# pinellolab/GRAFIMO

Measured on AMD Instinct MI355X. Metric: scored haplotype k-mers/sec, higher is better.
Workload: dtype int32

## Files before the change

### grafimo_amd/csrc/gfm_graph_fused.hpp

```cpp

constexpr int kMaxMM = 3;
struct GraphHit { int tile, score; long long q2k; };
constexpr int kHitWinShift = 56;
constexpr long long kHitWalkMask = (1ll << kHitWinShift) - 1;
struct Tile {
    long long p0, limit;
    int n_win, region;
    int i_lo, i_hi;
    int w_base, i_far;
};
constexpr int kTilePure = 1 << 8;
struct DelWin { int tile_k, i0; };
constexpr int kDelTileBits = 25;
__device__ __forceinline__ int del_tile(const DelWin &d) { return d.tile_k & ((1 << kDelTileBits) - 1); }
__device__ __forceinline__ int del_k(const DelWin &d) { return (int)((unsigned)d.tile_k >> kDelTileBits); }
struct HeavyWin {
    int tile_k, i0;
    int ns;
    unsigned item_base, n_chunks, rounds_per_chunk;
    long long walks;
    long long q_base;
    int jx, del_len;
};
constexpr long long kHeavyWalks = 64;
// ... 181 lines not shown

struct WinInfo {
    int i0, ns;
    long long walks;
    bool listed, simple;
    long long walks_b;
    int ns_b, jx, del_len;
};
template <class S>
__device__ __forceinline__ WinInfo classify_window(const GraphDev &g, const S &sites, long long p, int W, long long limit,
                                                   int i_lo, int i_hi)
{
    int lo = i_lo, hi = i_hi;
    while (lo < hi) {
        const int mid = (lo + hi) >> 1;
        if (sites.at(mid).pos < p) lo = mid + 1; else hi = mid;
    }
    WinInfo w{lo, 0, 1, false, false, 0, 0, 0, 0};
    bool over = false;
    const bool covered = g.n_dels > 0 && sites.covered(p, lo);
    w.listed = covered;
    int n_indel = 0, first_indel = -1;
    for (int i = lo;; ++i, ++w.ns) {
        const SiteRec r = sites.at(i);
        if (r.pos >= p + W) break;
        if (r.del_len || r.ins_len) {
            w.listed = true;
            if (n_indel++ == 0) first_indel = i;
        } else if (!over) {
            w.walks *= 1 + (r.n_alts & 3);
            over = w.walks > kFusedMaxWalks;
        }
    }
    bool ins_before = false;
    if (g.n_ins > 0) {
        for (int k = lo - 1; k >= i_lo; --k) {
            const SiteRec r = sites.at(k);
            if (r.pos != p - 1) break;
            if (r.ins_len > 0) { w.listed = true; ins_before = true; }
        }
        if (!w.listed && p + W > limit) { w.walks = 0; over = false; }
    }
    if (p + W > g.ref_len && !w.listed) w.walks = 0;
    if (w.listed && !covered && !ins_before && n_indel == 1 && !over) {
        const SiteRec d = sites.at(first_indel);
        if (d.del_len > 0) {
            const long long x = d.pos, len = d.del_len;
            bool ok = true, over_b = false;
            long long wb = 1;
            int nsb = 0;
            for (int i = lo;; ++i, ++nsb) {
                const SiteRec r = sites.at(i);
                if (r.pos >= p + W + len) break;
                if (r.del_len || r.ins_len) { if (i != first_indel) { ok = false; break; } continue; }
                if (r.pos > x && r.pos <= x + len) continue;
                if (!over_b) { wb *= 1 + (r.n_alts & 3); over_b = wb > kFusedMaxWalks; }
            }
            if (ok && !over_b) {
                w.simple = true;
                w.ns_b = nsb;
                w.jx = (int)(x - p);
                w.del_len = (int)len;
                const bool a_lives = p + W <= limit && p + W <= g.ref_len;
                const bool b_lives = a_lives && w.jx < W - 1 && p + W + len <= limit && p + W + len <= g.ref_len;
                if (!a_lives) w.walks = 0;
                w.walks_b = b_lives ? wb : 0;
                return w;
            }
        }
    }
    if (w.listed) w.walks = 0;
    else if (over) w.walks = -1;
    return w;
}

constexpr int kWaveQueue = 96;
constexpr int kOwnerSlots = 256;
template <int MM, bool LISTING, bool GENERAL> struct WaveLdsT {
    SiteRec rec[kWaveSites];
    uint2 winfo[kTileWin];
    unsigned wsc[MM][kTileWin];
    unsigned short incl[kTileWin];
    unsigned char owner[kOwnerSlots];
    unsigned char ref[kWaveRefBytes];
    int reach[GENERAL ? kWaveSites : 1];
    unsigned score_b[MM][GENERAL ? kTileWin : 1];
    unsigned sinfo[GENERAL ? kTileWin : 1];
    DelWin queue[(LISTING && GENERAL) ? kWaveQueue : 1];
};
__host__ __device__ constexpr int fused_tab_dwords(int MM, int W) { return (MM * W * 8 + 3) & ~3; }

#ifndef GFM_GRAPH_SCORE_MIN_WAVES
#define GFM_GRAPH_SCORE_MIN_WAVES 6
#endif
template <int MM, bool LISTING, bool GENERAL>
__global__ void __launch_bounds__(kFusedMaxWaves * 64, LISTING ? 1 : GFM_GRAPH_SCORE_MIN_WAVES)
graph_score_kernel(GraphDev g, FusedArgs a, const Tile *__restrict__ tiles, int tile_begin, int n_tiles,
                   DelWin *__restrict__ del_wins, int *__restrict__ del_count, int *__restrict__ overflow,
                   HeavyWin *__restrict__ heavy_wins, unsigned long long *__restrict__ heavy_ctl, int *__restrict__ plan_overflow_w)
{
    using WL = WaveLdsT<MM, LISTING, GENERAL>;
    extern __shared__ __attribute__((aligned(16))) unsigned char fused_lds[];
    const int W = a.W, W8 = W * 8;
    const int nw = (int)(blockDim.x >> 6), n_thr = (int)blockDim.x;
    unsigned *tab = reinterpret_cast<unsigned *>(fused_lds);
    WL *wl0 = reinterpret_cast<WL *>(tab + fused_tab_dwords(MM, W));
    WL *wl = wl0 + (threadIdx.x >> 6);
    unsigned long long *blk_rows = reinterpret_cast<unsigned long long *>(wl0 + nw);
    int *blk_q = reinterpret_cast<int *>(blk_rows + nw);
    unsigned *h = reinterpret_cast<unsigned *>(blk_q + nw + 4);
    const int tid = threadIdx.x, lane = tid & 63, wave = __builtin_amdgcn_readfirstlane(tid >> 6);
    int *next_tile = blk_q + nw + 1;
    unsigned long long rows_done = 0;
    int q_n = 0;
    unsigned long long acc_t[6] = {0, 0, 0, 0, 0, 0}, acc_n = 0;
#ifdef GFM_LAB
    unsigned ph_t[5] = {0, 0, 0, 0, 0};
#endif
    auto lap = [&](int slot, unsigned long long &t0) {
#ifdef GFM_LAB
        if (a.tile_log) {
            const unsigned long long t1 = wall_clock64();
            if (slot < 5) ph_t[slot] = (unsigned)(t1 - t0);
            t0 = t1;
            return;
        }
#endif
        if (!GFM_DBG(a)) return;
        const unsigned long long t1 = wall_clock64();
        acc_t[slot] += t1 - t0;
        t0 = t1;
    };
    static_assert(kWaveSites <= 64, "one staged record per lane");
    struct TilePf { SiteRec r0; int reach0; unsigned long long refw; };
    auto issue = [&](const Tile &t) {
        TilePf f{};
        const int staged = min(t.i_far - t.i_lo + 1, kWaveSites);
        if (lane < staged) {
            f.r0 = packed_site(g, t.i_lo + lane);
            if constexpr (GENERAL) {
                if (g.n_dels > 0 && !(t.n_win & kTilePure)) {
                    const int i = t.i_lo + lane;
                    const long long r = (i <= g.n_sites ? g.max_reach[i] : -1ll) - t.p0;
                    f.reach0 = (int)max(-1ll, min(r, 0x7fffffffll));
                }
            }
        }
        if (lane < kWaveRefBytes / 8) {
            const long long at = t.p0 + 8 * lane;
            unsigned long long v = 0x4e4e4e4e4e4e4e4eull;
            if (at + 8 <= g.ref_len + (long long)kReadPad) v = load_u64(g.ref + at);
            if (at + 8 > g.ref_len)
                for (int b = 0; b < 8; ++b)
                    if (at + b >= g.ref_len) v = (v & ~(0xffull << (8 * b))) | (0x4eull << (8 * b));
            f.refw = v;
        }
        return f;
    };
    auto commit = [&](const Tile &t, const TilePf &f) {
        const int staged = min(t.i_far - t.i_lo + 1, kWaveSites);
        if (lane < staged) {
            wl->rec[lane] = f.r0;
            if constexpr (GENERAL) wl->reach[lane] = f.reach0;
        }
        if (lane < kWaveRefBytes / 8) *reinterpret_cast<unsigned long long *>(wl->ref + 8 * lane) = f.refw;
    };
    auto tile_at = [&](int j) -> int {
        const long long at = (long long)tile_begin + (long long)blockIdx.x + (long long)j * (long long)gridDim.x;
        return at < (long long)n_tiles ? (int)at : n_tiles;
    };
    auto claim = [&]() -> int {
        int j = 0;
        if (lane == 0) j = atomicAdd(next_tile, 1);
        return tile_at(__builtin_amdgcn_readfirstlane(j));
    };
    static_assert(sizeof(Tile) == 40, "ten dwords");
    auto tile_ask = [&](int idx) -> unsigned {
        return lane < 10 ? reinterpret_cast<const unsigned *>(tiles + idx)[lane] : 0u;
    };
    auto tile_take = [&](unsigned dw) -> Tile {
        unsigned v[10];
#pragma unroll
        for (int k = 0; k < 10; ++k) v[k] = (unsigned)__builtin_amdgcn_readlane((int)dw, k);
        Tile t;
        t.p0 = (long long)(((unsigned long long)v[1] << 32) | v[0]);
        t.limit = (long long)(((unsigned long long)v[3] << 32) | v[2]);
        t.n_win = (int)v[4]; t.region = (int)v[5]; t.i_lo = (int)v[6]; t.i_hi = (int)v[7]; t.w_base = (int)v[8]; t.i_far = (int)v[9];
        return t;
    };
    Tile t_cur{}, t_nxt{};
    TilePf pf{};
    int ti = tile_at(wave), ti1 = n_tiles, ti2 = n_tiles;
    unsigned nxt_dw = ti < n_tiles ? tile_ask(ti) : 0u;
#pragma unroll
    for (int m = 0; m < MM; ++m)
        for (int i = tid; i < W8; i += n_thr) tab[m * W8 + i] = a.tab[m][i];
    for (int i = tid; i < a.slab_stride; i += n_thr) h[i] = 0u;
    if (tid == 0) { *next_tile = nw; next_tile[1] = 0; }
    if (ti < n_tiles) {
        t_cur = tile_take(nxt_dw);
        pf = issue(t_cur);
    }
    __syncthreads();
#ifndef GFM_GRAPH_HOLD1
    if (ti < n_tiles) {
        ti1 = claim();
        if (ti1 < n_tiles) nxt_dw = tile_ask(ti1);
    }
#endif
#ifdef GFM_LAB
    const unsigned long long dbg_t0 = a.tile_log ? wall_clock64() : 0ull;
#endif
    for (; ti < n_tiles; ti = ti1, ti1 = ti2) {
#ifdef GFM_LAB
        const unsigned long long tl_begin = a.tile_log ? wall_clock64() : 0ull;
#endif
#ifdef GFM_LAB
        unsigned long long tk0 = (GFM_DBG(a) || a.tile_log) ? wall_clock64() : 0ull, tk_tile = tk0;
#else
        unsigned long long tk0 = 0ull, tk_tile = 0ull;
#endif
        const Tile t = t_cur;
        commit(t, pf);
        const int my_pos = pf.r0.pos, my_alts = pf.r0.n_alts;
        __builtin_amdgcn_wave_barrier();
        ti2 = n_tiles;
#ifndef GFM_GRAPH_HOLD1
        if (ti1 < n_tiles) {
            t_nxt = tile_take(nxt_dw);
            pf = issue(t_nxt);
            t_cur = t_nxt;
            ti2 = claim();
            if (ti2 < n_tiles) nxt_dw = tile_ask(ti2);
        }
#else
        ti1 = claim();
        if (ti1 < n_tiles) nxt_dw = tile_ask(ti1);
#endif
        const int staged = min(t.i_far - t.i_lo + 1, kWaveSites);
        const int n_win = t.n_win & 0xff;
        lap(0, tk0);
        auto work = [&](const auto &sites, auto pure_tag) {
        constexpr bool PURE = decltype(pure_tag)::value;
        auto ref_at = [&](long long x) -> unsigned {
            const long long d = x - t.p0;
            if ((unsigned long long)d < (unsigned long long)kWaveRefBytes) return (unsigned)wl->ref[d];
            ColdArgs ka = cold_args();
            return x < ka->g.ref_len ? (unsigned)ka->g.ref[x] : (unsigned)'N';
        };
        const long long p = t.p0 + lane;
        bool listed = false;
        int i0 = t.i_lo, ns = 0, ns_b = 0, jx = 0, dlen = 0;
        int walks_a = 0, walks_b = 0;
        auto to_heavy = [&](long long n_walks, long long q_base, int ns_, int jx_, int del_len_) {
            if (!a.listing) return;
            const long long rounds = (n_walks + 63) >> 6;
            const unsigned n_chunks = (unsigned)min((long long)kHeavyMaxChunks, (rounds + kHeavyItemRounds - 1) / kHeavyItemRounds);
            ColdArgs ka = cold_args();
            const unsigned long long got = atomicAdd(ka->heavy_ctl, (1ull << 32) | (unsigned long long)n_chunks);
            const unsigned slot = (unsigned)(got >> 32), base = (unsigned)(got & 0xffffffffull);
            if (slot < (unsigned)kHeavyCap && (unsigned long long)base + n_chunks < 0xffffffffull) {
                ka->heavy_wins[slot] = HeavyWin{ti | (lane << kDelTileBits), i0, ns_, base, n_chunks,
                                            (unsigned)((rounds + n_chunks - 1) / n_chunks), n_walks, q_base, jx_, del_len_};
            } else {
                atomicMax(ka->overflow, 1);
                atomicMax(ka->plan_overflow_w, 1);
            }
        };
        if constexpr (PURE) {
            const int pi = (int)p, n_t = t.i_hi - t.i_lo;
            int before = 0, inside = 0;
            unsigned long long prod = 1;
            for (int s = 0; s < n_t; ++s) {
                const int spos = __builtin_amdgcn_readlane(my_pos, s);
                const int na = __builtin_amdgcn_readlane(my_alts, s) & 3;
                const bool bef = spos < pi, in = !bef && spos < pi + W;
                before += bef ? 1 : 0;
                inside += in ? 1 : 0;
                if (in && prod <= (unsigned long long)kFusedMaxWalks) prod *= (unsigned long long)(1 + na);
            }
            if (lane < n_win && !GFM_LAB_BIT(a, 4)) {
                i0 = t.i_lo + before;
                ns = inside;
                long long wlk = (p + W <= t.limit && p + W <= g.ref_len) ? (long long)prod : 0ll;
                if (wlk > kFusedMaxWalks) { atomicMax(cold_args()->overflow, 1); wlk = 0; }
                else if (wlk > kHeavyWalks) { to_heavy(wlk, 0, ns, 0, 0); wlk = 0; }
                walks_a = (int)wlk;
            }
        } else if (lane < n_win && !GFM_LAB_BIT(a, 4)) {
            WinInfo wi = classify_window(g, sites, p, W, t.limit, t.i_lo, t.i_hi);
            if (wi.walks < 0) { atomicMax(cold_args()->overflow, 1); wi.walks = 0; }
            i0 = wi.i0;
            if (wi.simple && (wi.ns_b > 255 || wi.del_len > 0xffff)) {
                wi.simple = false;
                wi.walks = 0;
                wi.walks_b = 0;
            }
            if (wi.i0 - t.i_lo > 0xffff) { atomicMax(cold_args()->overflow, 1); wi.walks = 0; wi.walks_b = 0; wi.listed = wi.simple = false; }
            const bool many = wi.walks + wi.walks_b > kHeavyWalks;
            if (wi.simple && many) {
                if (wi.ns <= 64 && wi.ns_b <= 64) {
                    if (wi.walks > 0) to_heavy(wi.walks, 0, wi.ns, 0, 0);
                    if (wi.walks_b > 0) to_heavy(wi.walks_b, wi.walks, wi.ns_b, wi.jx, wi.del_len);
                    wi.listed = false;
                } else {
                    wi.simple = false;
                }
                wi.walks = 0;
                wi.walks_b = 0;
            }
            listed = wi.listed && !wi.simple;
            if (!wi.listed && !wi.simple && many && wi.ns <= 64) {
                to_heavy(wi.walks, 0, wi.ns, 0, 0);
                wi.walks = 0;
            }
            ns = wi.ns; ns_b = wi.ns_b; jx = wi.jx; dlen = wi.del_len;
            walks_a = (int)wi.walks;
            walks_b = (int)wi.walks_b;
        }
        if (GFM_LAB_BIT(a, 4) && lane < n_win) walks_a = 1;
        lap(1, tk0);
        unsigned sc_a[MM];
#pragma unroll
        for (int m = 0; m < MM; ++m) sc_a[m] = 0u;
        int bad_a = 0;
        if (lane < n_win) {
            if (walks_a > 0 && !GFM_LAB_BIT(a, 2)) {
                int bad = 0;
                int j = 0;
                for (; j + 4 <= W; j += 4) {
                    unsigned c[4];
#pragma unroll
                    for (int u = 0; u < 4; ++u) c[u] = base_code(wl->ref[lane + j + u]);
#pragma unroll
                    for (int m = 0; m < MM; ++m) {
                        unsigned v[4];
#pragma unroll
                        for (int u = 0; u < 4; ++u) v[u] = tab[m * W8 + (j + u) * 8 + c[u]];
                        sc_a[m] += (v[0] + v[1]) + (v[2] + v[3]);
                    }
                    bad += (int)((c[0] >> 2) + (c[1] >> 2) + (c[2] >> 2) + (c[3] >> 2));
                }
                for (; j < W; ++j) {
                    const unsigned c = base_code(wl->ref[lane + j]);
#pragma unroll
                    for (int m = 0; m < MM; ++m) sc_a[m] += tab[m * W8 + j * 8 + c];
                    bad += (int)(c >> 2);
                }
                bad_a = bad;
            }
            if constexpr (!PURE) if (walks_b > 0) {
                unsigned sum[MM];
#pragma unroll
                for (int m = 0; m < MM; ++m) sum[m] = 0u;
                int bad = 0;
                if (lane + W + dlen <= kWaveRefBytes) {
                    const unsigned char *rb = wl->ref + lane;
                    int j = 0;
                    for (; j + 4 <= W; j += 4) {
                        unsigned c[4];
#pragma unroll
                        for (int u = 0; u < 4; ++u) c[u] = base_code(rb[j + u + (j + u > jx ? dlen : 0)]);
#pragma unroll
                        for (int m = 0; m < MM; ++m) {
                            unsigned v[4];
#pragma unroll
                            for (int u = 0; u < 4; ++u) v[u] = tab[m * W8 + (j + u) * 8 + c[u]];
                            sum[m] += (v[0] + v[1]) + (v[2] + v[3]);
                        }
                        bad += (int)((c[0] >> 2) + (c[1] >> 2) + (c[2] >> 2) + (c[3] >> 2));
                    }
                    for (; j < W; ++j) {
                        const unsigned c = base_code(rb[j + (j > jx ? dlen : 0)]);
#pragma unroll
                        for (int m = 0; m < MM; ++m) sum[m] += tab[m * W8 + j * 8 + c];
                        bad += (int)(c >> 2);
                    }
                } else {
                    for (int j = 0; j < W; ++j) {
                        const unsigned c = base_code(ref_at(p + j + (j > jx ? dlen : 0)));
#pragma unroll
                        for (int m = 0; m < MM; ++m) sum[m] += tab[m * W8 + j * 8 + c];
                        bad += (int)(c >> 2);
                    }
                }
#pragma unroll
                for (int m = 0; m < MM; ++m) wl->score_b[m][lane] = sum[m];
                wl->sinfo[lane] = (unsigned)bad | ((unsigned)jx << 8) | ((unsigned)dlen << 16);
            }
        }
        lap(2, tk0);
        {
            const bool has_ref = walks_a > 0;
            if (!GFM_LAB_BIT(a, 8)) {
#pragma unroll
                for (int m = 0; m < MM; ++m) {
                    const int s_f = bad_a ? a.min_val[m] : (int)(sc_a[m] & 0xffffu);
                    const int s_r = bad_a ? a.min_val[m] : (int)(sc_a[m] >> 16);
                    if (a.hnb[m] > 0) {
                        book_score_cold(a, m, h, has_ref, s_f);
                        if (!a.forward_only) book_score_cold(a, m, h, has_ref, s_r);
                    }
                    push_hits_cold(m, has_ref && s_f >= a.cutoff[m], ti, lane, 0, s_f);
                    if (!a.forward_only) push_hits_cold(m, has_ref && s_r >= a.cutoff[m], ti, lane, 1, s_r);
                }
            }
            rows_done += (unsigned long long)__popcll(__builtin_amdgcn_ballot_w64(has_ref)) * (a.forward_only ? 1ull : 2ull);
        }
        if constexpr (LISTING && !PURE) {
            const unsigned long long lm = __builtin_amdgcn_ballot_w64(listed);
            if (lm) {
                if (listed) wl->queue[q_n + __popcll(lm & ((1ull << lane) - 1ull))] = DelWin{ti | (lane << kDelTileBits), i0};
                q_n += __popcll(lm);
                if (q_n >= kWaveQueue - kTileWin) {
                    int base = 0;
                    if (lane == 0) base = atomicAdd(cold_args()->del_count, q_n);
                    base = __builtin_amdgcn_readfirstlane(base);
                    __builtin_amdgcn_wave_barrier();
                    { DelWin *dw = cold_args()->del_wins; for (int i = lane; i < q_n; i += 64) dw[base + i] = wl->queue[i]; }
                    q_n = 0;
                }
            }
        }
        const int nA = walks_a > 0 ? walks_a - 1 : 0;
        const int v_w = nA + walks_b;
        const int incl = wave_prefix_sum(v_w);
        int total = __builtin_amdgcn_readlane(incl, 63);
        if (GFM_LAB_BIT(a, 1)) total = 0;
        const bool owners = total < kOwnerSlots;
        if (total > 0) {
            wl->incl[lane] = (unsigned short)incl;
            if (owners)
                for (int x = incl - v_w; x < incl; ++x) wl->owner[x] = (unsigned char)lane;
            wl->winfo[lane] = uint2{(unsigned)(i0 - t.i_lo) | ((unsigned)ns << 16) | ((unsigned)ns_b << 24),
                                    (unsigned)bad_a | ((unsigned)walks_a << 7) | ((unsigned)(incl - v_w) << 14)};
#pragma unroll
            for (int m = 0; m < MM; ++m) wl->wsc[m][lane] = sc_a[m];
        }
        __builtin_amdgcn_wave_barrier();
        lap(3, tk0);
#ifdef GFM_GRAPH_HOLD1
        if (ti1 < n_tiles) {
            t_nxt = tile_take(nxt_dw);
            pf = issue(t_nxt);
            t_cur = t_nxt;
        }
#endif
        for (int base = 0; base < total; base += 64) {
            const int wt = base + lane;
            const bool live = wt < total;
            int k = 0;
            long long q = 0;
            unsigned sum[MM];
#pragma unroll
            for (int m = 0; m < MM; ++m) sum[m] = 0u;
            int bad = 0;
            if (live) {
                if (owners) {
                    k = wl->owner[wt];
                } else {
                    int lo = 0, hi = kTileWin - 1;
                    while (lo < hi) {
                        const int mid = (lo + hi) >> 1;
                        if ((int)wl->incl[mid] > wt) hi = mid; else lo = mid + 1;
                    }
                    k = lo;
                }
                const uint2 pw = wl->winfo[k];
                const int qq = wt - (int)(pw.y >> 14);
                const int wa = (int)((pw.y >> 7) & 0x7fu);
                const int nA_k = wa > 0 ? wa - 1 : 0;
                const bool jump = qq >= nA_k;
                const int i0k = t.i_lo + (int)(pw.x & 0xffffu);
                if (!jump) {
                    q = qq + 1;
#pragma unroll
                    for (int m = 0; m < MM; ++m) sum[m] = wl->wsc[m][k];
                    bad = (int)(pw.y & 0x7fu);
                    unsigned rest = (unsigned)q;
                    const int pk = (int)(t.p0 + k);
                    for (int s = (int)((pw.x >> 16) & 0xffu) - 1; s >= 0 && rest; --s) {
                        const SiteRec r = sites.at(i0k + s);
                        const int nall = (r.del_len | r.ins_len) ? 1 : 1 + (r.n_alts & 3);
                        const int al = take_digit32(rest, nall);
                        if (al) {
                            const int j = r.pos - pk;
                            const unsigned cr = base_code(wl->ref[k + j]), ca = base_code((unsigned)r.n_alts >> (8 * al));
#pragma unroll
                            for (int m = 0; m < MM; ++m) sum[m] += tab[m * W8 + j * 8 + ca] - tab[m * W8 + j * 8 + cr];
                            bad += (int)(ca >> 2) - (int)(cr >> 2);
                        }
                    }
                } else if constexpr (!PURE) {
                    q = (long long)wa + (qq - nA_k);
#pragma unroll
                    for (int m = 0; m < MM; ++m) sum[m] = wl->score_b[m][k];
                    const unsigned si = wl->sinfo[k];
                    bad = (int)(si & 0xffu);
                    unsigned rest = (unsigned)(qq - nA_k);
                    const long long pk = t.p0 + k;
                    const long long x = pk + (long long)((si >> 8) & 0xffu), len = (long long)(si >> 16);
                    for (int s = (int)(pw.x >> 24) - 1; s >= 0 && rest; --s) {
                        const SiteRec r = sites.at(i0k + s);
                        if (r.del_len | r.ins_len) continue;
                        if (r.pos > x && r.pos <= x + len) continue;
                        const int nall = 1 + (r.n_alts & 3);
                        const int al = take_digit32(rest, nall);
                        if (al) {
                            const int j = (int)(r.pos - pk) - (r.pos > x ? (int)len : 0);
                            const unsigned cr = base_code(ref_at(r.pos)), ca = base_code((unsigned)r.n_alts >> (8 * al));
#pragma unroll
                            for (int m = 0; m < MM; ++m) sum[m] += tab[m * W8 + j * 8 + ca] - tab[m * W8 + j * 8 + cr];
                            bad += (int)(ca >> 2) - (int)(cr >> 2);
                        }
                    }
                }
            }
            if (GFM_LAB_BIT(a, 8)) continue;
#pragma unroll
            for (int m = 0; m < MM; ++m) {
                const int s_f = bad ? a.min_val[m] : (int)(sum[m] & 0xffffu);
                const int s_r = bad ? a.min_val[m] : (int)(sum[m] >> 16);
                if (a.hnb[m] > 0) {
                    book_score_cold(a, m, h, live, s_f);
                    if (!a.forward_only) book_score_cold(a, m, h, live, s_r);
                }
                push_hits_cold(m, live && s_f >= a.cutoff[m], ti, k, 2 * q, s_f);
                if (!a.forward_only) push_hits_cold(m, live && s_r >= a.cutoff[m], ti, k, 2 * q + 1, s_r);
            }
        }
        rows_done += (unsigned long long)total * (a.forward_only ? 1ull : 2ull);
        };
        if constexpr (!GENERAL) {
            work(LdsTileSites{wl->rec, nullptr, t.p0, t.i_lo}, std::true_type{});
        } else {
            if (t.n_win & kTilePure) work(LdsTileSites{wl->rec, wl->reach, t.p0, t.i_lo}, std::true_type{});
            else if (t.i_far - t.i_lo + 1 <= kWaveSites) work(LdsTileSites{wl->rec, wl->reach, t.p0, t.i_lo}, std::false_type{});
            else {
                const GraphDev g_far = ((const ScoreKernArgs *)cold_args())->g;
                work(TileSites{g_far, wl->rec, wl->reach, t.p0, t.i_lo, staged}, std::false_type{});
            }
        }
        __builtin_amdgcn_wave_barrier();
        lap(4, tk0);
        lap(5, tk_tile);
#ifdef GFM_LAB
        if (a.tile_log && lane == 0 && !a.listing) {
            a.tile_log[ti] = (((wall_clock64() - tl_begin) & 0xffffffull) << 40) | (((tl_begin - dbg_t0) & 0xffffffull) << 16) | (blockIdx.x & 0xffffu);
            unsigned long long w = 0;
            for (int k = 0; k < 5; ++k) w |= (unsigned long long)min(ph_t[k], 4095u) << (12 * k);
            a.tile_log[n_tiles + ti] = w;
        }
#endif
        ++acc_n;
    }
    if (const int lw_items = cold_args()->a.lw_items; lw_items > 0) {
        ColdArgs ka = cold_args();
        const int n16 = ka->a.lw_pitch >> 4;
        for (;;) {
            int j = 0;
            if (lane == 0) j = atomicAdd(next_tile + 1, 1);
            const long long it = (long long)blockIdx.x + (long long)__builtin_amdgcn_readfirstlane(j) * (long long)gridDim.x;
            if (it >= (long long)lw_items) break;
            const size_t row = (size_t)it * 64 + (size_t)lane;
            const LwMeta me = ka->a.lw_meta[row];
            const bool live = me.tile_k >= 0;
            uint4 v[4];
#pragma unroll
            for (int c = 0; c < 4; ++c) v[c] = (c < n16 && live) ? ka->a.lw_kmers[row * (size_t)n16 + c] : uint4{0x41414141u, 0x41414141u, 0x41414141u, 0x41414141u};
            unsigned sum[MM];
#pragma unroll
            for (int m = 0; m < MM; ++m) sum[m] = 0u;
            int bad = 0;
#pragma unroll
            for (int c = 0; c < 4; ++c) {
                if (16 * c >= W) break;
                const unsigned dw[4] = {v[c].x, v[c].y, v[c].z, v[c].w};
#pragma unroll
                for (int u = 0; u < 16; ++u) {
                    const int jj = 16 * c + u;
                    if (jj < W) {
                        const unsigned cd = base_code((dw[u >> 2] >> (8 * (u & 3))) & 0xffu);
#pragma unroll
                        for (int m = 0; m < MM; ++m) sum[m] += tab[m * W8 + jj * 8 + cd];
                        bad += (int)(cd >> 2);
                    }
                }
            }
            const int w_tile = me.tile_k & ((1 << kDelTileBits) - 1), w_k = (int)((unsigned)me.tile_k >> kDelTileBits);
#pragma unroll
            for (int m = 0; m < MM; ++m) {
                const int s_f = bad ? a.min_val[m] : (int)(sum[m] & 0xffffu);
                const int s_r = bad ? a.min_val[m] : (int)(sum[m] >> 16);
                if (a.hnb[m] > 0) {
                    book_score_cold(a, m, h, live, s_f);
                    if (!a.forward_only) book_score_cold(a, m, h, live, s_r);
                }
                push_hits_cold(m, live && s_f >= a.cutoff[m], w_tile, w_k, 2 * me.q0, s_f);
                if (!a.forward_only) push_hits_cold(m, live && s_r >= a.cutoff[m], w_tile, w_k, 2 * me.q0 + 1, s_r);
            }
            rows_done += (unsigned long long)__popcll(__builtin_amdgcn_ballot_w64(live)) * (a.forward_only ? 1ull : 2ull);
        }
    }
    if (unsigned long long *dbg = GFM_DBG(a); dbg && lane == 0 && acc_n)
        for (int k = 0; k < 6; ++k) {
            atomicAdd(&dbg[8 + k], acc_t[k]);
            atomicMax(&dbg[24 + k], acc_t[k]);
            atomicAdd(&dbg[40 + k], acc_n);
        }
    if (lane == 0) { blk_rows[wave] = rows_done; blk_q[wave] = q_n; }
    __syncthreads();
    if (tid == 0) {
        if (!a.listing && blockIdx.x == 0 && *cold_args()->a.plan_overflow) atomicMax(cold_args()->overflow, 1);
        unsigned long long rows = 0;
        int left = 0;
        for (int k = 0; k < nw; ++k) { rows += blk_rows[k]; left += blk_q[k]; }
        if (rows) atomicAdd(cold_args()->a.n_rows, rows);
        blk_q[nw] = left ? atomicAdd(cold_args()->del_count, left) : 0;
    }
    __syncthreads();
    if constexpr (LISTING && GENERAL) {
        int at = blk_q[nw];
        for (int k = 0; k < wave; ++k) at += blk_q[k];
        { DelWin *dw = cold_args()->del_wins; for (int i = lane; i < q_n; i += 64) dw[at + i] = wl->queue[i]; }
    }
    { unsigned *slabs = cold_args()->a.slabs; for (int i = tid; i < a.slab_stride; i += n_thr) slabs[(size_t)blockIdx.x * a.slab_stride + i] = h[i]; }
}

struct ScoreEmit {
    const uint8_t *alt_bases, *ins_bases;
    const int *ins_off;
    uint8_t *fwd;
    int *src;
    static constexpr bool kWantsBases = true;
    __device__ void base(int j, long long x, int snp, int a, int)
    {
        src[j] = (int)x;
        if (snp >= 0 && a) { fwd[j] = alt_bases[(size_t)snp * kMaxAlts + (a - 1)]; src[j] = -1; }
    }
    __device__ void ins_base(int j, int site, int t) { fwd[j] = ins_bases[ins_off[site] + t]; src[j] = -1; }
    __device__ void took(int) {}
    __device__ void passed(int) {}
};


struct DelBatchRec {
    long long incl;
    int n_lay, pad;
    LayoutRec lay[kFusedLayouts];
};
struct DelItem { int batch, chunk, n_chunks, pad; };
constexpr int kDelItemRounds = 1, kDelMaxItems = 64;
constexpr int kDelExtraItems = 1 << 20, kDelMaxChunks = 1 << 18;

__global__ void __launch_bounds__(kFusedDelThreads)
graph_del_count_kernel(GraphDev g, int W, const Tile *__restrict__ tiles, const DelWin *__restrict__ del_wins,
                       const int *__restrict__ del_count, int *__restrict__ overflow, int *__restrict__ plan_overflow,
                       DelBatchRec *__restrict__ recs, DelItem *__restrict__ items, int *__restrict__ item_count,
                       int *__restrict__ extra_used, int *__restrict__ long_items)
{
    extern __shared__ __attribute__((aligned(16))) unsigned char fused_lds[];
    constexpr int T = kFusedDelThreads;
    SiteRec *cache = reinterpret_cast<SiteRec *>(fused_lds);
    const int lane = threadIdx.x;
    const int n_listed = *del_count;
    for (int batch = blockIdx.x; (long long)batch * T < n_listed; batch += gridDim.x) {
        __syncthreads();
        const int m = batch * T + lane;
        long long walks = 0;
        DelBatchRec rec{};
// ... 545 lines not shown
```

### grafimo_amd/csrc/graph_extract.hip

```cpp

#include <hip/hip_runtime.h>
#include <hip/hip_ext.h>

#include <cstdlib>
#include <hipcub/hipcub.hpp>

#include <algorithm>
#include <chrono>
#include <cstdint>
#include <cstdio>
#include <cstring>
#include <new>
#include <string>
#include <thread>
#include <vector>

#include "grafimo_hip.h"
#include "gfm_graph_host.hpp"

#define GFM_API extern "C" __attribute__((visibility("default")))
extern "C" void gfm_set_error_(const char *msg);

namespace {

// ... 1605 lines not shown
                               int *win_lo, int *win_nb, int *device, int *n_cu, const unsigned **d_ftab);

namespace {
constexpr int kFusedMaxBins[kMaxMM] = {16384, 8000, 5400};
#ifndef GFM_GRAPH_SMALL_BINS1
#define GFM_GRAPH_SMALL_BINS1 8000
#endif
constexpr int kFusedSmallBins[kMaxMM] = {GFM_GRAPH_SMALL_BINS1, 6000, 5000};
constexpr size_t kCuLdsBytes = 160 * 1024;

int site_lower_bound(const std::vector<int> &pos, int hint, long long target)
{
    const int n = (int)pos.size();
    if (hint > n) hint = n;
    if (hint > 0 && (long long)pos[(size_t)hint - 1] >= target) hint = 0;
    int step = 1, lo = hint, hi = hint;
    while (hi < n && (long long)pos[(size_t)hi] < target) { lo = hi + 1; hi += step; step <<= 1; }
    if (hi > n) hi = n;
    return (int)(std::lower_bound(pos.begin() + lo, pos.begin() + hi, target, [](int a, long long b) { return (long long)a < b; }) -
                 pos.begin());
}

struct KernelInfo { const void *fn = nullptr; int vgprs = 128; bool ready = false; };
int kernel_prepare(KernelInfo &k, const void *fn)
{
    if (k.ready) return GFM_OK;
    hipFuncAttributes at{};
    GX_TRY(hipFuncGetAttributes(&at, fn));
    GX_TRY(hipFuncSetAttribute(fn, hipFuncAttributeMaxDynamicSharedMemorySize, (int)kCuLdsBytes));
    k.fn = fn;
    k.vgprs = std::max(8, at.numRegs);
    k.ready = true;
    return GFM_OK;
}
struct Shape { int waves = 8, per_cu = 1; };
Shape pick_shape(int vgprs, size_t lds_fixed, size_t lds_per_wave)
{
    const int alloc = (vgprs + 7) & ~7;
    const int by_regs = std::max(1, std::min(8, 512 / std::max(8, alloc))) * 4;
    Shape best{};
    int best_waves = 0;
#ifdef GFM_LAB
    static const int force = [] { const char *e = std::getenv("GRAFIMO_FUSED_WAVES"); return e ? atoi(e) : 0; }();
#else
    constexpr int force = 0;
#endif
    for (int per_cu = 2; per_cu >= 1; --per_cu)
        for (int waves = kFusedMaxWaves; waves >= 4; waves -= 4) {
            if (force && waves != force) continue;
            if ((size_t)per_cu * (lds_fixed + (size_t)waves * lds_per_wave) > kCuLdsBytes) continue;
            if (per_cu * waves > by_regs) continue;
            if (per_cu * waves > best_waves) { best_waves = per_cu * waves; best = Shape{waves, per_cu}; }
        }
    if (best_waves == 0) best = Shape{4, 1};
    return best;
}

template <int MM> struct FusedKernels {
    static KernelInfo score[2][2], heavy, del_score;
};
template <int MM> KernelInfo FusedKernels<MM>::score[2][2];
template <int MM> KernelInfo FusedKernels<MM>::heavy;
template <int MM> KernelInfo FusedKernels<MM>::del_score;

struct FusedLaunch {
    gfm_graph *g;
    FusedPlan *P;
    FusedArgs a;
    hipStream_t st;
    int n_cu, n_motifs;
    bool listing, indels, with_hist;
    unsigned long long *heavy_ctl;
    int *overflow;
};

template <int MM> int launch_fused(FusedLaunch &L)
{
    gfm_graph *g = L.g;
    FusedPlan *P = L.P;
    FusedArgs &a = L.a;
    hipStream_t st = L.st;
    const int W = a.W, n_cu = L.n_cu;
    const size_t tab_bytes = sizeof(unsigned) * (size_t)fused_tab_dwords(MM, W), hist_bytes = sizeof(unsigned) * (size_t)a.slab_stride;
    using FK = FusedKernels<MM>;
    struct Part { int begin, end, grid; Shape sh; size_t lds; } part[2];
#ifdef GFM_LAB
    static const int split = [] { const char *e = std::getenv("GRAFIMO_FUSED_SPLIT"); return e ? atoi(e) : 0; }();
#else
    constexpr int split = 0;
#endif
    for (int general = 1; general >= 0; --general) {
        KernelInfo &ks = FK::score[L.listing ? 1 : 0][general];
        const void *fn = L.listing ? (general ? reinterpret_cast<const void *>(graph_score_kernel<MM, true, true>)
                                              : reinterpret_cast<const void *>(graph_score_kernel<MM, true, false>))
                                   : (general ? reinterpret_cast<const void *>(graph_score_kernel<MM, false, true>)
                                              : reinterpret_cast<const void *>(graph_score_kernel<MM, false, false>));
        if (const int rc = kernel_prepare(ks, fn)) return rc;
        const size_t wave_bytes = L.listing ? (general ? sizeof(WaveLdsT<MM, true, true>) : sizeof(WaveLdsT<MM, true, false>))
                                            : (general ? sizeof(WaveLdsT<MM, false, true>) : sizeof(WaveLdsT<MM, false, false>));
        Part &pt = part[general];
        pt.begin = general ? 0 : (split ? P->f_n_general : P->f_n_tiles);
        pt.end = general ? (split ? P->f_n_general : P->f_n_tiles) : P->f_n_tiles;
        pt.sh = pick_shape(ks.vgprs, tab_bytes + hist_bytes + 16, wave_bytes + sizeof(long long) + sizeof(int));
        const int n_t = pt.end - pt.begin;
        pt.grid = n_t > 0 ? std::max(1, std::min((n_t + pt.sh.waves - 1) / pt.sh.waves, pt.sh.per_cu * n_cu)) : 0;
        pt.lds = tab_bytes + (size_t)pt.sh.waves * wave_bytes + sizeof(long long) * (size_t)pt.sh.waves + sizeof(int) * (size_t)(pt.sh.waves + 4) + hist_bytes;
    }
    const int g1 = part[0].grid + part[1].grid;
    if (const int rc = kernel_prepare(FK::heavy, reinterpret_cast<const void *>(graph_heavy_kernel<MM>))) return rc;
    const Shape shh = pick_shape(FK::heavy.vgprs, tab_bytes + hist_bytes + 16, sizeof(HeavyLdsT<MM>) + sizeof(long long));
    const int g_heavy = shh.per_cu * n_cu;
    const size_t lds_h = tab_bytes + (size_t)shh.waves * sizeof(HeavyLdsT<MM>) + sizeof(long long) * (size_t)shh.waves + hist_bytes;
    GX_TRY(g->f_slabs.reserve((size_t)std::max(g1, g_heavy) * (size_t)std::max(1, a.slab_stride) + 1));
    a.slabs = g->f_slabs.p;
    auto launch_del_score = [&](hipStream_t on, int grid_cap, bool fill_cache) -> int {
        if (const int rc = kernel_prepare(FK::del_score, reinterpret_cast<const void *>(graph_del_score_kernel<MM>))) return rc;
        int pitch = ((W + 3) / 4) * 4;
        if ((pitch / 4) % 2 == 0) pitch += 4;
        const size_t lds_b = tab_bytes + sizeof(SiteRec) * kSiteCache * kFusedDelThreads +
                             sizeof(LayoutRec) * kFusedDelThreads * kFusedLayouts + 3 * sizeof(long long) * kFusedDelThreads +
                             3 * sizeof(int) * kFusedDelThreads + sizeof(int) * (size_t)kFusedDelThreads * W +
                             (size_t)kFusedDelThreads * pitch;
        const int per_cu = (int)std::max<size_t>(1, std::min<size_t>(8, (size_t)(150 * 1024) / lds_b));
        const int grid = grid_cap > 0 ? std::min(grid_cap, per_cu * n_cu) : per_cu * n_cu;
        hipLaunchKernelGGL((graph_del_score_kernel<MM>), dim3((unsigned)grid), dim3(kFusedDelThreads), lds_b, on, g->dev, a,
                           P->f_tiles.p, P->f_del_wins.p, P->f_flags.p + 1, P->f_del_recs.p, P->f_del_items.p, P->f_flags.p + 3,
                           pitch, fill_cache ? P->f_lw_kmers.p : nullptr, fill_cache ? P->f_lw_meta.p : nullptr, P->lw_pitch);
        return GFM_OK;
    };
#ifdef GFM_LAB
    static const bool serial = [] { const char *e = std::getenv("GRAFIMO_FUSED_BESIDE"); return !(e && *e == '1'); }();
#else
    constexpr bool serial = true;
#endif
    if (!P->items_known && P->items_asked) {
        if (hipEventQuery(P->ev_items) == hipSuccess) P->items_known = true;
        else (void)hipGetLastError();
    }
    const int n_items = P->items_known ? (int)(P->h_heavy_ctl[1] & 0xffffffffull) : -1;
    bool lw_fill = false;
    if (!L.listing && L.indels && P->lw_state == 0 && P->items_known) {
        static const size_t kLwCacheBytes = [] {
            const char *e = std::getenv("GRAFIMO_FUSED_WALK_CACHE_BYTES");
            return e ? (size_t)strtoull(e, nullptr, 10) : (size_t)256 << 20;
        }();
        const int pitch16 = ((W + 15) / 16) * 16;
        const size_t rows = (size_t)std::max(n_items, 0) * kFusedDelThreads;
        if (n_items > 0 && (int)(P->h_heavy_ctl[2] & 0xffffffffull) == 0 && rows * ((size_t)pitch16 + sizeof(LwMeta)) <= kLwCacheBytes) {
            GX_TRY(P->f_lw_kmers.reserve(rows * (size_t)pitch16 + 16));
            GX_TRY(P->f_lw_meta.reserve(rows + 1));
            GX_TRY(hipMemsetAsync(P->f_lw_meta.p, 0xff, rows * sizeof(LwMeta), st));
            P->lw_pitch = pitch16;
            P->lw_items = n_items;
            lw_fill = true;
        } else {
            P->lw_state = -1;
        }
    }
    const bool lw_cached = !L.listing && P->lw_state == 1;
    if (lw_cached) {
        a.lw_kmers = reinterpret_cast<const uint4 *>(P->f_lw_kmers.p);
        a.lw_meta = P->f_lw_meta.p;
        a.lw_items = P->lw_items;
        a.lw_pitch = P->lw_pitch;
    }
    const bool beside = split == 2 && part[0].grid > 0 && part[1].grid > 0;
    const bool del_beside = !L.listing && L.indels && !serial && n_items > 0;
    const bool del_none = !L.listing && (n_items == 0 || lw_cached);
    if (L.indels) {
        const size_t n_batches = ((size_t)P->f_general_windows + kFusedDelThreads - 1) / kFusedDelThreads;
        GX_TRY(P->f_del_recs.reserve(n_batches * kFusedDelThreads + 1));
        GX_TRY(P->f_del_items.reserve(n_batches * kDelMaxItems + (size_t)kDelExtraItems + 1));
    }
    if (beside || del_beside) {
        GX_TRY(hipEventRecord(g->ev_fork, st));
        GX_TRY(hipStreamWaitEvent(g->side, g->ev_fork, 0));
    }
    const bool timed = g->prof_on && g->prof_n < gfm_graph::kProfSlots;
    const bool timed_on_dispatch = timed && part[0].grid == 0 && !beside;
    if (timed && !timed_on_dispatch) GX_TRY(hipEventRecord(g->prof_ev[2 * g->prof_n], st));
    for (int general = 1; general >= 0; --general) {
        const Part &pt = part[general];
        if (pt.grid == 0) continue;
        hipStream_t st = (beside && general) ? g->side : L.st;
        FusedArgs ap = a;
        ap.slabs = a.slabs + (general ? (size_t)0 : (size_t)part[1].grid * (size_t)a.slab_stride);
        if (!general && part[1].grid > 0) ap.lw_items = 0;
        const dim3 grid((unsigned)pt.grid), block((unsigned)pt.sh.waves * 64);
#define GFM_LAUNCH_SCORE(LST, GEN)                                                                                              \
// ... 396 lines not shown
```

Measured before the change: 219.5 billion.

## Score k-mers with pair-of-bases LDS table and dword-packed reference reads

Replaces the per-position PWM table in LDS with a table indexed by pairs of adjacent positions (64 entries per pair), so each window needs half as many table lookups. Reference bytes are read four at a time as dwords using alignbyte, and base codes and the N-count are derived with bit tricks. Deletion-branch windows merge pre- and post-deletion bytes with a byte mask. The price is a larger LDS table (8x bigger per position pair), which can lower occupancy, plus extra setup work at kernel start.

```diff
diff --git a/grafimo_amd/csrc/gfm_graph_fused.hpp b/grafimo_amd/csrc/gfm_graph_fused.hpp
--- a/grafimo_amd/csrc/gfm_graph_fused.hpp
+++ b/grafimo_amd/csrc/gfm_graph_fused.hpp
@@ -287,13 +287,36 @@
     unsigned wsc[MM][kTileWin];
     unsigned short incl[kTileWin];
     unsigned char owner[kOwnerSlots];
-    unsigned char ref[kWaveRefBytes];
+    unsigned char ref[kWaveRefBytes + 8];
     int reach[GENERAL ? kWaveSites : 1];
     unsigned score_b[MM][GENERAL ? kTileWin : 1];
     unsigned sinfo[GENERAL ? kTileWin : 1];
     DelWin queue[(LISTING && GENERAL) ? kWaveQueue : 1];
 };
 __host__ __device__ constexpr int fused_tab_dwords(int MM, int W) { return (MM * W * 8 + 3) & ~3; }
+__host__ __device__ constexpr int fused_ptab_dwords(int MM, int W) { return (W + 1) / 2 * 64 * MM; }
+__device__ __forceinline__ int pair_at(int j, unsigned c, int MM) { return ((j >> 1) * 64 + (int)(c << (3 * (j & 1)))) * MM; }
+template <int MM>
+__device__ __forceinline__ void pair_dword(const unsigned *ptab, unsigned x, int k, int W, unsigned (&sum)[MM], int &bad)
+{
+    const unsigned y = (x >> 1) & 0x07070707u, z = y | (y >> 5);
+    const int n = W - 4 * k;
+    bad += __popc(x & 0x08080808u & (n >= 4 ? 0xffffffffu : (1u << (8 * n)) - 1u));
+    const unsigned *e0 = ptab + ((2 * k) * 64 + (int)(z & 63u)) * MM;
+    if (n > 2) {
+        const unsigned *e1 = ptab + ((2 * k + 1) * 64 + (int)((z >> 16) & 63u)) * MM;
+#pragma unroll
+        for (int m = 0; m < MM; ++m) sum[m] += e0[m] + e1[m];
+    } else {
+#pragma unroll
+        for (int m = 0; m < MM; ++m) sum[m] += e0[m];
+    }
+}
+__device__ __forceinline__ unsigned lds_dword_at(const unsigned char *buf, int o)
+{
+    const unsigned *w = reinterpret_cast<const unsigned *>(buf) + (o >> 2);
+    return __builtin_amdgcn_alignbyte(w[1], w[0], (unsigned)(o & 3));
+}
 
 #ifndef GFM_GRAPH_SCORE_MIN_WAVES
 #define GFM_GRAPH_SCORE_MIN_WAVES 6
@@ -306,10 +329,10 @@
 {
     using WL = WaveLdsT<MM, LISTING, GENERAL>;
     extern __shared__ __attribute__((aligned(16))) unsigned char fused_lds[];
-    const int W = a.W, W8 = W * 8;
+    const int W = a.W;
     const int nw = (int)(blockDim.x >> 6), n_thr = (int)blockDim.x;
-    unsigned *tab = reinterpret_cast<unsigned *>(fused_lds);
-    WL *wl0 = reinterpret_cast<WL *>(tab + fused_tab_dwords(MM, W));
+    unsigned *ptab = reinterpret_cast<unsigned *>(fused_lds);
+    WL *wl0 = reinterpret_cast<WL *>(ptab + fused_ptab_dwords(MM, W));
     WL *wl = wl0 + (threadIdx.x >> 6);
     unsigned long long *blk_rows = reinterpret_cast<unsigned long long *>(wl0 + nw);
     int *blk_q = reinterpret_cast<int *>(blk_rows + nw);
@@ -397,9 +420,17 @@
     TilePf pf{};
     int ti = tile_at(wave), ti1 = n_tiles, ti2 = n_tiles;
     unsigned nxt_dw = ti < n_tiles ? tile_ask(ti) : 0u;
-#pragma unroll
-    for (int m = 0; m < MM; ++m)
-        for (int i = tid; i < W8; i += n_thr) tab[m * W8 + i] = a.tab[m][i];
+    {
+        const int n_pe = fused_ptab_dwords(1, W);
+#pragma unroll
+        for (int m = 0; m < MM; ++m)
+            for (int e = tid; e < n_pe; e += n_thr) {
+                const int j = (e >> 6) * 2;
+                unsigned v = a.tab[m][j * 8 + (e & 7)];
+                if (j + 1 < W) v += a.tab[m][(j + 1) * 8 + ((e >> 3) & 7)];
+                ptab[e * MM + m] = v;
+            }
+    }
     for (int i = tid; i < a.slab_stride; i += n_thr) h[i] = 0u;
     if (tid == 0) { *next_tile = nw; next_tile[1] = 0; }
     if (ti < n_tiles) {
@@ -531,27 +562,12 @@
         int bad_a = 0;
         if (lane < n_win) {
             if (walks_a > 0 && !GFM_LAB_BIT(a, 2)) {
+                const unsigned *rw = reinterpret_cast<const unsigned *>(wl->ref) + (lane >> 2);
+                const unsigned sh = (unsigned)(lane & 3);
                 int bad = 0;
-                int j = 0;
-                for (; j + 4 <= W; j += 4) {
-                    unsigned c[4];
-#pragma unroll
-                    for (int u = 0; u < 4; ++u) c[u] = base_code(wl->ref[lane + j + u]);
-#pragma unroll
-                    for (int m = 0; m < MM; ++m) {
-                        unsigned v[4];
-#pragma unroll
-                        for (int u = 0; u < 4; ++u) v[u] = tab[m * W8 + (j + u) * 8 + c[u]];
-                        sc_a[m] += (v[0] + v[1]) + (v[2] + v[3]);
-                    }
-                    bad += (int)((c[0] >> 2) + (c[1] >> 2) + (c[2] >> 2) + (c[3] >> 2));
-                }
-                for (; j < W; ++j) {
-                    const unsigned c = base_code(wl->ref[lane + j]);
-#pragma unroll
-                    for (int m = 0; m < MM; ++m) sc_a[m] += tab[m * W8 + j * 8 + c];
-                    bad += (int)(c >> 2);
-                }
+                const int nd = (W + 3) >> 2;
+#pragma unroll 4
+                for (int k = 0; k < nd; ++k) pair_dword<MM>(ptab, __builtin_amdgcn_alignbyte(rw[k + 1], rw[k], sh), k, W, sc_a, bad);
                 bad_a = bad;
             }
             if constexpr (!PURE) if (walks_b > 0) {
@@ -560,33 +576,21 @@
                 for (int m = 0; m < MM; ++m) sum[m] = 0u;
                 int bad = 0;
                 if (lane + W + dlen <= kWaveRefBytes) {
-                    const unsigned char *rb = wl->ref + lane;
-                    int j = 0;
-                    for (; j + 4 <= W; j += 4) {
-                        unsigned c[4];
-#pragma unroll
-                        for (int u = 0; u < 4; ++u) c[u] = base_code(rb[j + u + (j + u > jx ? dlen : 0)]);
-#pragma unroll
-                        for (int m = 0; m < MM; ++m) {
-                            unsigned v[4];
-#pragma unroll
-                            for (int u = 0; u < 4; ++u) v[u] = tab[m * W8 + (j + u) * 8 + c[u]];
-                            sum[m] += (v[0] + v[1]) + (v[2] + v[3]);
-                        }
-                        bad += (int)((c[0] >> 2) + (c[1] >> 2) + (c[2] >> 2) + (c[3] >> 2));
-                    }
-                    for (; j < W; ++j) {
-                        const unsigned c = base_code(rb[j + (j > jx ? dlen : 0)]);
-#pragma unroll
-                        for (int m = 0; m < MM; ++m) sum[m] += tab[m * W8 + j * 8 + c];
-                        bad += (int)(c >> 2);
+                    const int nd = (W + 3) >> 2;
+#pragma unroll 2
+                    for (int k = 0; k < nd; ++k) {
+                        const int o = lane + 4 * k, nlo = jx + 1 - 4 * k;
+                        const unsigned lo = lds_dword_at(wl->ref, o), hi = lds_dword_at(wl->ref, o + dlen);
+                        const unsigned keep = nlo >= 4 ? 0xffffffffu : (nlo <= 0 ? 0u : (1u << (8 * nlo)) - 1u);
+                        pair_dword<MM>(ptab, (lo & keep) | (hi & ~keep), k, W, sum, bad);
                     }
                 } else {
-                    for (int j = 0; j < W; ++j) {
-                        const unsigned c = base_code(ref_at(p + j + (j > jx ? dlen : 0)));
-#pragma unroll
-                        for (int m = 0; m < MM; ++m) sum[m] += tab[m * W8 + j * 8 + c];
-                        bad += (int)(c >> 2);
+                    for (int j = 0; j < W; j += 2) {
+                        const unsigned c0 = base_code(ref_at(p + j + (j > jx ? dlen : 0)));
+                        const unsigned c1 = j + 1 < W ? base_code(ref_at(p + j + 1 + (j + 1 > jx ? dlen : 0))) : 0u;
+#pragma unroll
+                        for (int m = 0; m < MM; ++m) sum[m] += ptab[((j >> 1) * 64 + (int)(c0 | (c1 << 3))) * MM + m];
+                        bad += (int)((c0 >> 2) + (c1 >> 2));
                     }
                 }
 #pragma unroll
@@ -691,8 +695,9 @@
                         if (al) {
                             const int j = r.pos - pk;
                             const unsigned cr = base_code(wl->ref[k + j]), ca = base_code((unsigned)r.n_alts >> (8 * al));
-#pragma unroll
-                            for (int m = 0; m < MM; ++m) sum[m] += tab[m * W8 + j * 8 + ca] - tab[m * W8 + j * 8 + cr];
+                            const unsigned *ea = ptab + pair_at(j, ca, MM), *er = ptab + pair_at(j, cr, MM);
+#pragma unroll
+                            for (int m = 0; m < MM; ++m) sum[m] += ea[m] - er[m];
                             bad += (int)(ca >> 2) - (int)(cr >> 2);
                         }
                     }
@@ -714,8 +719,9 @@
                         if (al) {
                             const int j = (int)(r.pos - pk) - (r.pos > x ? (int)len : 0);
                             const unsigned cr = base_code(ref_at(r.pos)), ca = base_code((unsigned)r.n_alts >> (8 * al));
-#pragma unroll
-                            for (int m = 0; m < MM; ++m) sum[m] += tab[m * W8 + j * 8 + ca] - tab[m * W8 + j * 8 + cr];
+                            const unsigned *ea = ptab + pair_at(j, ca, MM), *er = ptab + pair_at(j, cr, MM);
+#pragma unroll
+                            for (int m = 0; m < MM; ++m) sum[m] += ea[m] - er[m];
                             bad += (int)(ca >> 2) - (int)(cr >> 2);
                         }
                     }
@@ -782,15 +788,8 @@
                 if (16 * c >= W) break;
                 const unsigned dw[4] = {v[c].x, v[c].y, v[c].z, v[c].w};
 #pragma unroll
-                for (int u = 0; u < 16; ++u) {
-                    const int jj = 16 * c + u;
-                    if (jj < W) {
-                        const unsigned cd = base_code((dw[u >> 2] >> (8 * (u & 3))) & 0xffu);
-#pragma unroll
-                        for (int m = 0; m < MM; ++m) sum[m] += tab[m * W8 + jj * 8 + cd];
-                        bad += (int)(cd >> 2);
-                    }
-                }
+                for (int u = 0; u < 4; ++u)
+                    if (16 * c + 4 * u < W) pair_dword<MM>(ptab, dw[u], 4 * c + u, W, sum, bad);
             }
             const int w_tile = me.tile_k & ((1 << kDelTileBits) - 1), w_k = (int)((unsigned)me.tile_k >> kDelTileBits);
 #pragma unroll
diff --git a/grafimo_amd/csrc/graph_extract.hip b/grafimo_amd/csrc/graph_extract.hip
--- a/grafimo_amd/csrc/graph_extract.hip
+++ b/grafimo_amd/csrc/graph_extract.hip
@@ -1711,6 +1711,7 @@
     hipStream_t st = L.st;
     const int W = a.W, n_cu = L.n_cu;
     const size_t tab_bytes = sizeof(unsigned) * (size_t)fused_tab_dwords(MM, W), hist_bytes = sizeof(unsigned) * (size_t)a.slab_stride;
+    const size_t ptab_bytes = sizeof(unsigned) * (size_t)fused_ptab_dwords(MM, W);
     using FK = FusedKernels<MM>;
     struct Part { int begin, end, grid; Shape sh; size_t lds; } part[2];
 #ifdef GFM_LAB
@@ -1730,10 +1731,10 @@
         Part &pt = part[general];
         pt.begin = general ? 0 : (split ? P->f_n_general : P->f_n_tiles);
         pt.end = general ? (split ? P->f_n_general : P->f_n_tiles) : P->f_n_tiles;
-        pt.sh = pick_shape(ks.vgprs, tab_bytes + hist_bytes + 16, wave_bytes + sizeof(long long) + sizeof(int));
+        pt.sh = pick_shape(ks.vgprs, ptab_bytes + hist_bytes + 16, wave_bytes + sizeof(long long) + sizeof(int));
         const int n_t = pt.end - pt.begin;
         pt.grid = n_t > 0 ? std::max(1, std::min((n_t + pt.sh.waves - 1) / pt.sh.waves, pt.sh.per_cu * n_cu)) : 0;
-        pt.lds = tab_bytes + (size_t)pt.sh.waves * wave_bytes + sizeof(long long) * (size_t)pt.sh.waves + sizeof(int) * (size_t)(pt.sh.waves + 4) + hist_bytes;
+        pt.lds = ptab_bytes + (size_t)pt.sh.waves * wave_bytes + sizeof(long long) * (size_t)pt.sh.waves + sizeof(int) * (size_t)(pt.sh.waves + 4) + hist_bytes;
     }
     const int g1 = part[0].grid + part[1].grid;
     if (const int rc = kernel_prepare(FK::heavy, reinterpret_cast<const void *>(graph_heavy_kernel<MM>))) return rc;
```

Result: no change. 218.0 billion, median of 6 (-0.7%).
